# kzampog/cilantro

Hardware: NVIDIA H100
Metric: icp_correspondences_per_sec (higher is better)
Workload: dtype f32

## Files before the change

### cilantro_b200/capi.py

```python
import ctypes as C
import os
import weakref

import numpy as np

_HERE = os.path.dirname(os.path.abspath(__file__))
LIB_PATH = os.environ.get("CILANTRO_B200_LIB", os.path.join(_HERE, "libcilantro_b200.so"))

CB_OK = 0


class CbError(RuntimeError):
    pass


class IcpParams(C.Structure):
    _fields_ = [
        ("metric", C.c_int32),
        ("max_iter", C.c_int32),
        ("tol", C.c_float),
        ("max_d2", C.c_float),
        ("w_pt", C.c_float),
        ("w_pl", C.c_float),
        ("max_opt_iter", C.c_int32),
# ... 611 lines not shown
        n = lib().cb_icp_iteration_times(self.h, _p(times), C.c_int(times.shape[0]))
        return {
            "T": np.array(list(res.T), np.float32).reshape(3, 4),
            "iterations": int(res.iterations),
            "last_delta": float(res.last_delta),
            "converged": bool(res.converged),
            "num_corr": int(res.num_corr),
            "gpu_ms_total": float(res.gpu_ms_total),
            "gpu_ms_search": float(res.gpu_ms_search),
            "iter_ms": times[:max(n, 0)],
            "kernel_launches": int(res.kernel_launches),
        }

    def accumulate(self, T, **kw):
        prm = kw.pop("params", None) or icp_params(**kw)
        sums = np.zeros(28, np.float64)
        nv = _check(lib().cb_icp_accumulate(self.h, C.byref(prm), _p(_T(T)), _p(sums), C.c_int(28)))
        return sums[:nv]

    def correspondences(self):
        n = self.src.n + self.dst.n
        i1 = np.empty(n, np.uint64)
        i2 = np.empty(n, np.uint64)
        v = np.empty(n, np.float32)
        cnt = C.c_size_t()
        _check(lib().cb_icp_correspondences(self.h, _p(i1), _p(i2), _p(v), C.byref(cnt)))
        c = cnt.value
        return i1[:c].astype(np.int64), i2[:c].astype(np.int64), v[:c]

    def loop_cache(self):
        T = np.empty((3, 4), np.float32)
        near = np.empty(self.src.n, np.int64)
        cnt = C.c_uint64()
        _check(lib().cb_icp_loop_cache(self.h, _p(T), _p(near), C.byref(cnt)))
        return T, near, int(cnt.value)

    def residuals(self, T, **kw):
        prm = kw.pop("params", None) or icp_params(**kw)
        out = np.empty(self.src.n, np.float32)
        _check(lib().cb_icp_residuals(self.h, C.byref(prm), _p(_T(T)), _p(out)))
        return out


def solve_kabsch_moments(sums16):
    s = np.ascontiguousarray(sums16, np.float64)
    T = np.empty((3, 4), np.float32)
    ok = _check(lib().cb_solve_kabsch_moments(_p(s), _p(T)))
    return T, bool(ok)


def solve_gauss_newton(sums28, T_in=None):
    s = np.ascontiguousarray(sums28, np.float64)
    Ti = identity() if T_in is None else _T(T_in)
    To = np.empty((3, 4), np.float32)
    dn = C.c_float()
    _check(lib().cb_solve_gauss_newton(_p(s), _p(Ti), _p(To), C.byref(dn)))
    return To, dn.value


def solve_rotation(L):
    L = np.ascontiguousarray(L, np.float32).reshape(3, 3)
    R = np.empty((3, 3), np.float32)
    _check(lib().cb_solve_rotation(_p(L), _p(R)))
    return R


def compose(A, B):
    out = np.empty((3, 4), np.float32)
# ... 315 lines not shown
```

### cilantro_b200/csrc/capi_core.cu

```cuda
#include "cb_internal.hpp"
#include "icp_kernels.cuh"
#include "stats_kernels.cuh"
#include "host_solve.hpp"
#include "icp_object.hpp"
#include <atomic>
#include <cstdlib>
#include <cstring>
#include <cfloat>
#include <cmath>
#include <algorithm>
#include <vector>
#include <string>

namespace cb {

static thread_local std::string g_err;

void set_error(const char* fmt, ...) {
  char buf[1024];
  va_list ap;
  va_start(ap, fmt);
  vsnprintf(buf, sizeof(buf), fmt, ap);
  va_end(ap);
  g_err = buf;
// ... 875 lines not shown
    a.n_src = (uint32_t)ns;
    a.T = to_rigid(icp->T_search);
    a.Tin = to_rigid(nullptr);
    a.max_d2 = icp->max_d2_search;
    a.nn_pos = icp->d_nn_pos;
    a.nn_d2 = icp->d_nn_d2;
    CB_TRY(launch_icp_pass(ctx, a, kModeKnn, true, false, false));
    icp->nn_stored = true;
  }
  DeviceScope sc(ctx);
  int* d_first = nullptr;
  float* d_val = nullptr;
  CB_TRY(sc.alloc(&d_first, ns));
  CB_TRY(sc.alloc(&d_val, ns));
  CB_TRY(launch_translate_matches(ctx, icp->d_nn_pos, icp->d_nn_d2, icp->src->d_pts, icp->dst->d_pts, (uint32_t)ns, d_first,
                                  d_val));
  std::vector<int> first(ns);
  std::vector<float> val(ns);
  CB_CUDA(cudaMemcpyAsync(first.data(), d_first, ns * sizeof(int), cudaMemcpyDeviceToHost, ctx->stream));
  CB_CUDA(cudaMemcpyAsync(val.data(), d_val, ns * sizeof(float), cudaMemcpyDeviceToHost, ctx->stream));
  CB_CUDA(cudaStreamSynchronize(ctx->stream));
  size_t k = 0;
  for (size_t i = 0; i < ns; i++) {
    if (first[i] < 0) continue;
    if (index_first) index_first[k] = (uint64_t)first[i] + icp->dst->index_offset;
    if (index_second) index_second[k] = (uint64_t)i + icp->src->index_offset;
    if (value) value[k] = val[i];
    ++k;
  }
  *count = k;
  return CB_OK;
}

int cb_icp_loop_cache(cb_icp* icp, float* T_search12, int64_t* nearest, uint64_t* searched_last) {
  CB_CHECK(icp, CB_ERR_INVALID, "null argument");
  CB_CHECK(icp->loop_last && icp->h_state, CB_ERR_INVALID, "the last cb_icp_estimate did not run on the device loop");
  cb_context* ctx = icp->ctx;
  CB_CUDA(cudaSetDevice(ctx->device));
  const size_t ns = icp->src->n;
  if (T_search12) std::memcpy(T_search12, icp->T_search, sizeof(icp->T_search));
  if (searched_last) *searched_last = icp->searched_last;
  if (nearest && ns) {
    DeviceScope sc(ctx);
    int* d_first = nullptr;
    CB_TRY(sc.alloc(&d_first, ns));
    CB_TRY(launch_translate_matches(ctx, icp->d_nn_pos, nullptr, icp->src->d_pts, icp->dst->d_pts, (uint32_t)ns, d_first,
                                    nullptr));
    std::vector<int> first(ns);
    CB_CUDA(cudaMemcpyAsync(first.data(), d_first, ns * sizeof(int), cudaMemcpyDeviceToHost, ctx->stream));
    CB_CUDA(cudaStreamSynchronize(ctx->stream));
    for (size_t i = 0; i < ns; i++) nearest[i] = first[i] < 0 ? -1 : (int64_t)first[i] + (int64_t)icp->dst->index_offset;
  }
  return CB_OK;
}

int cb_icp_residuals(cb_icp* icp, const cb_icp_params* prm, const float* T12, float* out) {
  CB_CHECK(icp && prm && T12 && out, CB_ERR_INVALID, "null argument");
  cb_context* ctx = icp->ctx;
  CB_CUDA(cudaSetDevice(ctx->device));
  const size_t ns = icp->src->n;
  if (ns == 0) return CB_OK;
  CB_CHECK(prm->metric == CB_ICP_POINT_TO_POINT || icp->dst->d_nrm || icp->dst->n == 0, CB_ERR_INVALID,
           "dst has no normals");
  DeviceScope scope(ctx);
  float* d_out = nullptr;
  CB_TRY(scope.alloc(&d_out, ns));
  CB_TRY(launch_residuals(ctx, grid_view(icp->dst), icp->src->d_pts,
                          prm->metric == CB_ICP_COMBINED ? icp->src->d_nrm : nullptr, (uint32_t)ns, to_rigid(T12),
                          prm->metric, prm->w_pt, prm->w_pl, d_out));
  CB_CUDA(cudaMemcpyAsync(out, d_out, ns * sizeof(float), cudaMemcpyDeviceToHost, ctx->stream));
  CB_CUDA(cudaStreamSynchronize(ctx->stream));
  return CB_OK;
}

}
```

### cilantro_b200/csrc/icp_loop.cu

```cuda
#include "cache_rule.hpp"
#include "icp_accumulate.cuh"
#include "icp_kernels.cuh"
#include "icp_object.hpp"
#include "reduce.cuh"
#include "solve_core.hpp"
#include "solve_warp.cuh"
#include "warp_search_wide.cuh"
#include <algorithm>
#include <cmath>
#include <cstdlib>
#include <cstring>

namespace cb {

namespace {

constexpr int kBlock = kReduceBlock;

struct LoopArgs {
  GridView dst;
  const float4* src_pts;
  const float4* src_nrm;
  uint32_t n_src;
  float max_d2, w_pt, w_pl, tol;
  int wk_pt, wk_pl;
  float wc_pt, wc_pl;
  float dm[3];
  float src_mean[3];
  int has_pt, has_pl;
  int bail;
  int* cache_pos;
  float* cache_r;
  float slack_first, slack_min, slack_max;
  LoopState* st;
  ReduceScratch rs;
  int trace;
};

struct BlockCtx {
  Rigid T, Tp;
  float dm[3], sm[3];
  float w_pt, w_pl;
  int wk_pt, wk_pl;
  float wc_pt, wc_pl;
  int have_prev, done;
};

__device__ __forceinline__ Rigid rigid_from_t12_dev(const float* T12) {
  Rigid r;
#pragma unroll
  for (int i = 0; i < 3; i++) {
#pragma unroll
    for (int j = 0; j < 3; j++) r.r[i * 3 + j] = __ldcg(T12 + i * 4 + j);
    r.t[i] = __ldcg(T12 + i * 4 + 3);
  }
  return r;
}

template <int MODE>
__device__ __forceinline__ void loop_solve(const LoopArgs* ap, const BlockCtx* cxp, const double* s, int late,
                                        unsigned long long seq) {
  const LoopArgs& a = *ap;
  const BlockCtx& cx = *cxp;
  LoopState* st = a.st;
  if (late) {
    st->error = CB_ERR_NCCL;
// ... 20 lines not shown
    }
  }
  sc::reorthonormalize(Titer);
  sc::compose(Titer, T, Tn);
  const float delta = sc::update_norm(Titer);
  for (int i = 0; i < 12; i++) {
    st->T_prev[i] = T[i];
    st->T[i] = Tn[i];
    st->Titer[i] = Titer[i];
  }
  for (int i = 0; i < 28; i++) st->sums[i] = (i < (MODE == kModeP2PCentered ? kP2PValues : kCombinedValues)) ? s[i] : 0.0;
  st->last_delta = delta;
  st->iters = st->iters + 1;
  st->n_corr = s[0];
  st->have_prev = 1;
  st->xseq = seq;
  st->searched_last = st->searched_cur;
  st->searched_cur = 0ull;
  if (delta < a.tol) st->done = 1;
  if (a.trace) {
    st->trace[(st->iters - 1) & 63][3] = global_timer_ns();
    st->trace[st->iters & 63][5] = 0ull;
  }
  __threadfence();
}

struct ChunkPair {
  uint32_t i;
  int pos;
  float qx, qy, qz;
  float d2;
};

constexpr unsigned int kColdGroup = 1, kWarmGroup = 2;
template <bool kCold>
__device__ __forceinline__ ChunkPair search_chunk_body(const LoopArgs& a, const BlockCtx& cx, WideSearchSmem* wsm,
                                                       bool act, uint32_t i) {
  ChunkPair cp;
  cp.i = i;
  cp.pos = -1;
  cp.qx = cp.qy = cp.qz = 0.f;
  cp.d2 = 0.f;
  float slack = a.slack_first;
  int sd = -1;
  if (act) {
    const float4 s = __ldg(a.src_pts + cp.i);
    rule::transform_point(cx.T, s.x, s.y, s.z, cp.qx, cp.qy, cp.qz);
    if (!kCold) {
      float ox, oy, oz;
      rule::transform_point(cx.Tp, s.x, s.y, s.z, ox, oy, oz);
      const float ex = __fsub_rn(cp.qx, ox), ey = __fsub_rn(cp.qy, oy), ez = __fsub_rn(cp.qz, oz);
      const float dl = __fsqrt_ru(__fmaf_ru(ez, ez, __fmaf_ru(ey, ey, __fmul_ru(ex, ex))));
      slack = fminf(fmaxf(__fmul_rn(2.f, dl), a.slack_min), a.slack_max);
      sd = a.cache_pos[cp.i];
    }
  }
  const WideBest wb = warp_grid_nearest_wide<kCold ? kColdGroup : kWarmGroup>(a.dst, *wsm, act, cp.qx, cp.qy, cp.qz, a.max_d2, sd, slack);
  if (act) {
    cp.pos = (wb.idx >= 0 && wb.d2 < a.max_d2) ? wb.pos : -1;
    cp.d2 = wb.d2;
    a.cache_pos[cp.i] = cp.pos;
    a.cache_r[cp.i] = rule::cache_radius(wb.D2);
  }
  return cp;
}

__device__ __noinline__ void search_chunk_far(const LoopArgs* ap, const BlockCtx* cxp, WideSearchSmem* wsm, bool act,
                                              uint32_t i, ChunkPair* out) {
  *out = search_chunk_body<false>(*ap, *cxp, wsm, act, i);
}

__device__ __forceinline__ void pdl_wait() { asm volatile("griddepcontrol.wait;" ::: "memory"); }
__device__ __forceinline__ void pdl_launch_dependents() { asm volatile("griddepcontrol.launch_dependents;" ::: "memory"); }

__device__ __forceinline__ void load_block_ctx(const LoopArgs& a, BlockCtx& cx) {
  cx.done = __ldcg(&a.st->done);
  cx.have_prev = __ldcg(&a.st->have_prev);
  cx.T = rigid_from_t12_dev(a.st->T);
  cx.Tp = rigid_from_t12_dev(a.st->T_prev);
  float smx, smy, smz;
  rule::transform_point(cx.T, a.src_mean[0], a.src_mean[1], a.src_mean[2], smx, smy, smz);
  cx.sm[0] = smx; cx.sm[1] = smy; cx.sm[2] = smz;
  cx.dm[0] = a.dm[0]; cx.dm[1] = a.dm[1]; cx.dm[2] = a.dm[2];
  cx.w_pt = a.w_pt;
  cx.w_pl = a.w_pl;
  cx.wk_pt = a.wk_pt;
  cx.wk_pl = a.wk_pl;
  cx.wc_pt = a.wc_pt;
  cx.wc_pl = a.wc_pl;
}

__host__ __device__ constexpr int pipe_qpt(bool normals) { return normals ? 2 : 1; }
__host__ __device__ constexpr int pipe_min_blocks(bool normals) { return normals ? 2 : 4; }

__device__ __forceinline__ uint32_t smem_u32(const void* p) { return (uint32_t)__cvta_generic_to_shared(p); }
__device__ __forceinline__ void cp_async_16_cg(void* dst_smem, const void* src) {
  asm volatile("cp.async.cg.shared.global [%0], [%1], 16;" ::"r"(smem_u32(dst_smem)), "l"(src) : "memory");
}
__device__ __forceinline__ void cp_async_16_ca(void* dst_smem, const void* src) {
  asm volatile("cp.async.ca.shared.global [%0], [%1], 16;" ::"r"(smem_u32(dst_smem)), "l"(src) : "memory");
}
__device__ __forceinline__ void cp_async_4(void* dst_smem, const void* src) {
// ... 140 lines not shown
      const unsigned int mm = __ballot_sync(0xffffffffu, miss);
      const unsigned int at = queued + __popc(mm & ((1u << lane) - 1u));
      if (miss && at < 32u) wq[at] = i;
      queued += __popc(mm);
      if (queued >= 32u) {
        search_queued(32u);
        queued -= 32u;
        if (miss && at >= 32u) wq[at - 32u] = i;
      }
    }
    abuf = abuf1;
    bbuf ^= 1;
  }
  cp_async_wait<0>();
  if (queued > 0u) search_queued(queued);
  if (lane == 0 && searched > 0u) {
    atomicAdd(&a.st->searched_cur, (unsigned long long)searched);
    if (a.trace) atomicAdd(&a.st->trace[__ldcg(&a.st->iters) & 63][4], (unsigned long long)searched);
  }
  if (a.trace && lane == 0) atomicMax(&a.st->trace[__ldcg(&a.st->iters) & 63][5], global_timer_ns());
  warp_sum_to_slot<NV, true>(acc, rsm);
  double tot = 0;
  if (!grid_reduce_slots_tail<NV>(a.rs, rsm, tot)) return;
  if (lane < NV) a.rs.result[lane] = tot;
  if (a.trace && lane == 0) a.st->trace[__ldcg(&a.st->iters) & 63][1] = global_timer_ns();
}

constexpr int kSearchMinBlocks = 4;

template <int MODE>
__global__ void __launch_bounds__(kBlock, kSearchMinBlocks) icp_search_kernel(const __grid_constant__ LoopArgs a) {
  constexpr int NV = (MODE == kModeP2PCentered) ? kP2PValues : kCombinedValues;
  __shared__ BlockCtx cx;
  __shared__ WideSearchSmem wsm[kBlock / 32];
  __shared__ AsyncReduceSmem<NV> rsm;

  const unsigned int tid = threadIdx.x, lane = tid & 31u, warp = tid >> 5;
  const uint32_t base = blockIdx.x * kBlock;
  pdl_wait();
  pdl_launch_dependents();
  if (tid == 0) {
    rsm.arrived = 0u;
    load_block_ctx(a, cx);
  }
  __syncthreads();
  if (cx.done) return;
  const int trace_slot = a.trace ? (__ldcg(&a.st->iters) & 63) : 0;
  if (a.trace && blockIdx.x == 0 && tid == 0) {
    a.st->trace[trace_slot][0] = global_timer_ns();
    a.st->trace[trace_slot][4] = 0ull;
  }
  const unsigned int total = (base < a.n_src) ? min((uint32_t)kBlock, a.n_src - base) : 0u;
  if (tid == 0 && total > 0) {
    atomicAdd(&a.st->searched_cur, (unsigned long long)total);
    if (a.trace) atomicAdd(&a.st->trace[trace_slot][4], (unsigned long long)total);
  }
  double acc[NV];
#pragma unroll
  for (int v = 0; v < NV; v++) acc[v] = 0.0;
  if ((tid & ~31u) < total) {
    const ChunkPair cp = search_chunk_body<true>(a, cx, &wsm[warp], tid < total, base + tid);
    if (cp.pos >= 0) {
      const float4 dp = __ldg(a.dst.pts + cp.pos);
      accumulate_pair<MODE, true>(
          acc, cx, a.has_pt != 0, a.has_pl != 0, dp, cp.qx, cp.qy, cp.qz, a.src_nrm != nullptr,
          [&] { return __ldg(a.dst.nrm + cp.pos); }, [&] { return __ldg(a.src_nrm + cp.i); }, cp.d2);
    }
  }
  if (a.trace && lane == 0) atomicMax(&a.st->trace[trace_slot][5], global_timer_ns());
  double tot = 0;
  if (!grid_reduce_async_tail<NV>(acc, a.rs, rsm, tot)) return;
  if (lane < NV) a.rs.result[lane] = tot;
  if (a.trace && lane == 0) a.st->trace[trace_slot][1] = global_timer_ns();
}

template <int MODE>
__global__ void __launch_bounds__(32, 1) icp_finish_kernel(const __grid_constant__ LoopArgs a) {
  constexpr int NV = (MODE == kModeP2PCentered) ? kP2PValues : kCombinedValues;
  __shared__ BlockCtx cx;
  __shared__ double sbuf[kCombinedValues + 8];
  static_assert(NV + 2 <= kExchangeVals, "row of the fused exchange");
  const unsigned int lane = threadIdx.x;
  pdl_wait();
  pdl_launch_dependents();
  if (lane == 0) load_block_ctx(a, cx);
  __syncwarp();
  if (cx.done) return;
  const int trace_slot = a.trace ? (__ldcg(&a.st->iters) & 63) : 0;
  double tot = (lane < NV) ? __ldcg(a.rs.result + lane) : 0.0;
  if (lane == NV) tot = (double)__ldcg(&a.st->searched_cur);
  if (lane == NV + 1) tot = (double)a.n_src;
  bool late = false;
  const unsigned long long seq = __ldcg(&a.st->xseq) + 1ull;
  if (a.rs.ex.enabled && a.rs.ex.world > 1) {
    Exchange ex = a.rs.ex;
    ex.seq = seq;
    tot = exchange_rows<NV + 2>(tot, ex, (int)lane, &late);
  }
  if (lane == NV) a.st->searched_all = tot;
  if (lane == NV + 1) a.st->queries_all = tot;
  if (a.trace && lane == 0) a.st->trace[trace_slot][2] = global_timer_ns();
  if (lane < NV) sbuf[lane] = tot;
  __syncwarp();
  if constexpr (MODE == kModeCombined) {
    double x[6];
    solve6_warp(sbuf, (int)lane, x);
    if (lane == 0)
#pragma unroll
      for (int i = 0; i < 6; i++) sbuf[kCombinedValues + i] = x[i];
    __syncwarp();
  }
  if (lane == 0) loop_solve<MODE>(&a, &cx, sbuf, late ? 1 : 0, seq);
}

}

constexpr float kSlackFirst = 0.20f, kSlackMin = 0.02f, kSlackMax = 0.30f;
constexpr int kBatch = 16;
constexpr int kFirstBatch = 4;
constexpr int kBridgeBatch = 2;
constexpr double kGiveUpShare = 0.15;

template <class Kernel>
static cudaError_t launch_pdl(Kernel k, int blocks, int threads, size_t smem, cudaStream_t stream, const LoopArgs& a) {
  cudaLaunchConfig_t cfg;
  std::memset(&cfg, 0, sizeof(cfg));
  cfg.gridDim = dim3((unsigned)blocks);
  cfg.blockDim = dim3((unsigned)threads);
  cfg.dynamicSmemBytes = smem;
  cfg.stream = stream;
  cudaLaunchAttribute attr[1];
  attr[0].id = cudaLaunchAttributeProgrammaticStreamSerialization;
  attr[0].val.programmaticStreamSerializationAllowed = 1;
  cfg.attrs = attr;
  cfg.numAttrs = 1;
  return cudaLaunchKernelEx(&cfg, k, a);
}

template <int MODE>
static int enqueue_iteration(cb_context* ctx, const LoopArgs& a, int it, int blocks_cold, int blocks_cached) {
  if (it == 0)
    CB_CUDA(launch_pdl(icp_search_kernel<MODE>, blocks_cold, kBlock, 0, ctx->stream, a));
  else
    CB_CUDA(launch_pdl(icp_cached_pipe_kernel<MODE>, blocks_cached, kBlock, sizeof(PipeSmem<MODE == kModeCombined>),
                       ctx->stream, a));
  CB_CUDA(launch_pdl(icp_finish_kernel<MODE>, 1, 32, 0, ctx->stream, a));
  ctx->launches += 2;
  return CB_OK;
}

// ... 6 lines not shown
  if (!icp->d_state) CB_TRY(icp->mem.alloc(&icp->d_state, 1));
  if (!icp->h_state) CB_TRY(icp->mem.alloc_host(&icp->h_state, 1));
  while (timing != 0 && (int)icp->events.size() < 2 * max_iter) {
    cudaEvent_t e;
    CB_CUDA(cudaEventCreate(&e));
    icp->events.push_back(e);
  }
  const size_t ns = icp->src->n;
  LoopArgs a;
  std::memset(&a, 0, sizeof(a));
  a.dst = grid_view(icp->dst);
  a.src_pts = icp->src->d_pts;
  a.src_nrm = (prm->metric == CB_ICP_COMBINED) ? icp->src->d_nrm : nullptr;
  a.n_src = (uint32_t)ns;
  a.max_d2 = prm->max_d2;
  a.w_pt = prm->w_pt;
  a.w_pl = prm->w_pl;
  a.wk_pt = prm->pt_weight_kind == CB_WEIGHT_RBF;
  a.wk_pl = prm->pl_weight_kind == CB_WEIGHT_RBF;
  a.wc_pt = prm->pt_weight_coeff;
  a.wc_pl = prm->pl_weight_coeff;
  a.tol = prm->tol;
  for (int r = 0; r < 3; r++) {
    a.dm[r] = icp->dst_mean[r];
    a.src_mean[r] = icp->src_mean[r];
  }
  const bool dst_has_normals = icp->dst->d_nrm != nullptr;
  a.has_pt = prm->w_pt > 0.f;
  a.has_pl = (prm->w_pl > 0.f) && dst_has_normals;
  a.bail = (prm->w_pl > 0.f) && !dst_has_normals;
  a.cache_pos = icp->d_nn_pos;
  a.cache_r = icp->d_nn_d2;
  const float h = 1.0f / a.dst.inv_h;
  a.slack_first = kSlackFirst * h;
  a.slack_min = kSlackMin * h;
  a.slack_max = kSlackMax * h;
  a.st = icp->d_state;
  static const bool trace = getenv("CB_LOOP_TRACE") != nullptr;
  a.trace = trace ? 1 : 0;
  const int blocks_cold = std::max(1, (int)((ns + kBlock - 1) / kBlock));
  static bool attr_set_dev[64] = {};
  static int resident_dev[64][2] = {};
  bool& attr_set = attr_set_dev[ctx->device & 63];
  int* resident = resident_dev[ctx->device & 63];
  if (!attr_set) {
    CB_CUDA(cudaFuncSetAttribute(icp_cached_pipe_kernel<kModeP2PCentered>, cudaFuncAttributeMaxDynamicSharedMemorySize,
                                 (int)sizeof(PipeSmem<false>)));
    CB_CUDA(cudaFuncSetAttribute(icp_cached_pipe_kernel<kModeCombined>, cudaFuncAttributeMaxDynamicSharedMemorySize,
                                 (int)sizeof(PipeSmem<true>)));
    CB_CUDA(cudaFuncSetAttribute(icp_cached_pipe_kernel<kModeP2PCentered>, cudaFuncAttributePreferredSharedMemoryCarveout,
                                 (int)cudaSharedmemCarveoutMaxShared));
    CB_CUDA(cudaFuncSetAttribute(icp_cached_pipe_kernel<kModeCombined>, cudaFuncAttributePreferredSharedMemoryCarveout,
                                 (int)cudaSharedmemCarveoutMaxShared));
    CB_CUDA(cudaOccupancyMaxActiveBlocksPerMultiprocessor(&resident[0], icp_cached_pipe_kernel<kModeP2PCentered>, kBlock,
                                                          sizeof(PipeSmem<false>)));
    CB_CUDA(cudaOccupancyMaxActiveBlocksPerMultiprocessor(&resident[1], icp_cached_pipe_kernel<kModeCombined>, kBlock,
                                                          sizeof(PipeSmem<true>)));
    attr_set = true;
  }
  const bool p2p = prm->metric == CB_ICP_POINT_TO_POINT;
  const int per_sm = std::max(1, resident[p2p ? 0 : 1]);
  const size_t tile = (size_t)pipe_qpt(!p2p) * kBlock;
  const int blocks_cached = std::max(1, std::min(ctx->sm_count * per_sm, (int)((ns + tile - 1) / tile)));
  CB_TRY(get_reduce_scratch(ctx, blocks_cold, kMaxValues, &a.rs));
  Exchange ex;
  std::memset(&ex, 0, sizeof(ex));
  const bool fused = ctx->world > 1 && arm_exchange(ctx, &ex);
  if (fused) ctx->seq -= 1;
  if (ctx->world > 1 && !fused) {
    set_error("the device-resident ICP loop needs the fused exchange (cb_comm_ipc_attach) when world > 1");
    return CB_ERR_UNSUPPORTED;
  }
  a.rs.ex = ex;
  ctx->pass_armed = false;

  LoopState* hs = icp->h_state;
  std::memset(hs, 0, sizeof(*hs));
  std::memcpy(hs->T, prm->T_init, sizeof(hs->T));
  std::memcpy(hs->T_prev, prm->T_init, sizeof(hs->T));
  hs->last_delta = INFINITY;
  hs->xseq = ctx->seq;
  CB_CUDA(cudaMemcpyAsync(icp->d_state, hs, sizeof(*hs), cudaMemcpyHostToDevice, ctx->stream));

  int issued = 0;
  if (!icp->h_state2) CB_TRY(icp->mem.alloc_host(&icp->h_state2, 1));
  for (int e = 0; e < 2; ++e)
    if (!icp->batch_ev[e]) CB_CUDA(cudaEventCreateWithFlags(&icp->batch_ev[e], cudaEventDisableTiming));
  LoopState* hbuf[2] = {icp->h_state, icp->h_state2};
  int enq = 0, checked = 0;
  auto enqueue_batch = [&](int n) -> int {
    for (int k = 0; k < n; ++k) {
      if (prm->flush_l2) CB_TRY(cb_context_flush_l2(ctx));
      if (timing) CB_CUDA(cudaEventRecord(icp->events[2 * (issued + k)], ctx->stream));
// ... 78 lines not shown
```

### cilantro_b200/csrc/nn_search.cuh

```cuda
#pragma once
#include "cache_rule.hpp"
#include "cb_internal.hpp"

namespace cb {

struct Rigid {
  float r[9];
  float t[3];
};

inline Rigid rigid_from_t12(const float* T12) {
  Rigid r;
  for (int i = 0; i < 3; i++) {
    for (int j = 0; j < 3; j++) r.r[i * 3 + j] = T12 ? T12[i * 4 + j] : (i == j ? 1.f : 0.f);
    r.t[i] = T12 ? T12[i * 4 + 3] : 0.f;
  }
  return r;
}

__device__ __forceinline__ float sum3(float a0, float a1, float a2) { return __fadd_rn(a0, __fadd_rn(a1, a2)); }

__device__ __forceinline__ void rotate_rigid(const Rigid& T, float x, float y, float z, float& qx, float& qy,
                                             float& qz) {
  qx = sum3(__fmul_rn(T.r[0], x), __fmul_rn(T.r[1], y), __fmul_rn(T.r[2], z));
// ... 83 lines not shown
      }
    }
  } else {
    scan_batched(pts, b, e, qx, qy, qz, [&](float r, uint32_t j) {
      if (r < best.d2) {
        best.d2 = r;
        best.pos = (int)j;
      } else if (r == best.d2 && (int)j != skip_pos) {
        best.tie = true;
      }
    });
  }
}

__device__ __forceinline__ float slab_gap(float f, int c, int r) {
  float g = 0.f;
  if (r > c) g = (float)r - f;
  if (r < c) g = f - (float)(r + 1);
  g -= kCellMargin;
  return g > 0.f ? g : 0.f;
}

__device__ __forceinline__ bool open_face_gap(const GridView& g, const QueryCell& c, int kk, float& gap) {
  float cover = 3.0e38f;
  bool any = false;
  if (c.cx - kk > 0) { cover = fminf(cover, c.fx - (float)(c.cx - kk)); any = true; }
  if (c.cx + kk < g.nx - 1) { cover = fminf(cover, (float)(c.cx + kk + 1) - c.fx); any = true; }
  if (c.cy - kk > 0) { cover = fminf(cover, c.fy - (float)(c.cy - kk)); any = true; }
  if (c.cy + kk < g.ny - 1) { cover = fminf(cover, (float)(c.cy + kk + 1) - c.fy); any = true; }
  if (c.cz - kk > 0) { cover = fminf(cover, c.fz - (float)(c.cz - kk)); any = true; }
  if (c.cz + kk < g.nz - 1) { cover = fminf(cover, (float)(c.cz + kk + 1) - c.fz); any = true; }
  gap = cover - kCellMargin;
  return any;
}

}

#include "far_sweep.cuh"

namespace cb {

template <bool kExact>
__device__ __forceinline__ Best grid_nearest_impl(const GridView& g, float qx, float qy, float qz, float max_d2) {
  Best best = no_best(max_d2);
  if (g.n == 0) return best;
  if (!(fabsf(qx) + fabsf(qy) + fabsf(qz) < 3.0e38f)) return best;

  const QueryCell c = query_cell(g, qx, qy, qz);
  const int cx = c.cx, cy = c.cy, cz = c.cz;
  const float hs2 = g.hs2;
  const int k0 = first_shell(g, c);
  int k = k0;
  if (k0 == 0) {
    const int xm = max(cx - 1, 0), xp = min(cx + 1, g.nx - 1);
    const uint32_t cbase = ((uint32_t)cz * (uint32_t)g.ny + (uint32_t)cy) * (uint32_t)g.nx;
    const uint32_t s0 = __ldg(g.cell_start + cbase + xm), s1 = __ldg(g.cell_start + cbase + cx);
    const uint32_t s2 = __ldg(g.cell_start + cbase + cx + 1), s3 = __ldg(g.cell_start + cbase + xp + 1);
    constexpr int kDy[8] = {-1, 1, 0, 0, -1, 1, -1, 1};
    constexpr int kDz[8] = {0, 0, -1, 1, -1, -1, 1, 1};
    uint32_t rb[8], re[8];
#pragma unroll
    for (int t = 0; t < 8; ++t) {
      const int ry = cy + kDy[t], rz = cz + kDz[t];
      const bool valid = (ry >= 0) & (ry < g.ny) & (rz >= 0) & (rz < g.nz);
      const uint32_t base = valid ? ((uint32_t)rz * (uint32_t)g.ny + (uint32_t)ry) * (uint32_t)g.nx : cbase;
      const uint32_t b = __ldg(g.cell_start + base + xm), e = __ldg(g.cell_start + base + xp + 1);
// ... 104 lines not shown
```

### cilantro_b200/csrc/warp_search_wide.cuh

```cuda
#pragma once
#include "warp_search.cuh"

namespace cb {

struct WideSearchSmem : WarpQueue {
  unsigned int sec[32];
};
static_assert(sizeof(WideSearchSmem) <= 3456, "WideSearchSmem must not grow");

struct WideBest {
  float d2;
  int idx;
  int pos;
  float D2;
};

__device__ __forceinline__ void two_smallest(float r, int j, float& b1, int& p1, float& b2) {
  if (r < b1) {
    b2 = b1;
    b1 = r;
    p1 = j;
  } else {
    b2 = fminf(b2, r);
  }
}

__device__ __forceinline__ void scan_range_two(const float4* __restrict__ pts, uint32_t b, uint32_t e, float qx, float qy,
                                               float qz, float& b1, int& p1, float& b2, int skip) {
  scan_batched(pts, b, e, qx, qy, qz, [&](float r, uint32_t j) {
    if ((int)j != skip) two_smallest(r, (int)j, b1, p1, b2);
  });
}

__device__ __forceinline__ void merge_region(WideSearchSmem& sm, unsigned int owner, float l1, int lp, float l2,
                                             float max_d2) {
  constexpr float kInf = 3.402823466e+38f;
  float loser = l1;
  if (l1 < max_d2) {
    const unsigned long long key = pack_key(l1, (unsigned int)lp);
    const unsigned long long old = atomicMin(&sm.key[owner], key);
    const float od2 = __uint_as_float((unsigned int)(old >> 32));
    loser = ((unsigned int)(old & 0xffffffffull) == 0xffffffffu) ? kInf : fmaxf(od2, l1);
  }
  atomicMin(&sm.sec[owner], __float_as_uint(fminf(l2, loser)));
}

template <unsigned int kGroup>
__device__ __forceinline__ WideBest warp_grid_nearest_wide(const GridView& g, WideSearchSmem& sm, bool active, float qx,
                                                           float qy, float qz, float max_d2, int warm_pos, float slack) {
  const unsigned int lane = threadIdx.x & 31;
  const unsigned int lt_mask = (1u << lane) - 1u;
  constexpr float kInf = 3.402823466e+38f;
  WideBest out;
  out.d2 = max_d2;
  out.idx = -1;
  out.pos = -1;
  out.D2 = 0.f;

  const QueryCell c = query_cell(g, qx, qy, qz);
  const bool inside = active && g.n > 0 && c.cx >= 0 && c.cx < g.nx && c.cy >= 0 && c.cy < g.ny && c.cz >= 0 && c.cz < g.nz;
  bool slow = active && g.n > 0 && !inside;

  float b1 = kInf, b2 = kInf;
  int p1 = -1;
  if (inside && warm_pos >= 0) {
    const float4 p = __ldg(g.pts + warm_pos);
    b1 = rule::contract_d2(qx, qy, qz, p.x, p.y, p.z);
    p1 = warm_pos;
  }
  sm.q[lane] = make_float4(qx, qy, qz, 0.f);
  __syncwarp();

  unsigned int count = 0;
  float wide2 = 0.f;
  {
    const uint32_t cbase = inside ? ((uint32_t)c.cz * (uint32_t)g.ny + (uint32_t)c.cy) * (uint32_t)g.nx : 0u;
    uint32_t s1 = 0, s2 = 0;
// ... 18 lines not shown
    for (int t = 0; t < 10; ++t) {
      bool need;
      uint32_t first;
      uint32_t ncells;
      if (t == 0) {
        need = inside && c.cx > 0 && (gxl * gxl * g.hs2 <= wide2);
        first = cbase + (uint32_t)(c.cx - 1);
        ncells = 1;
      } else if (t == 1) {
        need = inside && c.cx < g.nx - 1 && (gxr * gxr * g.hs2 <= wide2);
        first = cbase + (uint32_t)(c.cx + 1);
        ncells = 1;
      } else {
        const int ry = c.cy + kDy[t - 2], rz = c.cz + kDz[t - 2];
        const bool valid = inside && ry >= 0 && ry < g.ny && rz >= 0 && rz < g.nz;
        need = valid && ((gy2[kDy[t - 2] + 1] + gz2[kDz[t - 2] + 1]) * g.hs2 <= wide2);
        first = ((uint32_t)rz * (uint32_t)g.ny + (uint32_t)ry) * (uint32_t)g.nx + (uint32_t)xm;
        ncells = (uint32_t)(xp - xm + 1);
      }
      const unsigned int m = __ballot_sync(0xffffffffu, need);
      if (need) sm.item[count + __popc(m & lt_mask)] = make_uint2(first, (ncells << 8) | lane);
      count += __popc(m);
    }
    if (b1 < max_d2) {
      sm.key[lane] = pack_key(b1, (unsigned int)p1);
      sm.sec[lane] = __float_as_uint(b2);
    } else {
      sm.key[lane] = pack_key(max_d2, 0xffffffffu);
      sm.sec[lane] = __float_as_uint(b1);
    }
  }
  __syncwarp();

  static_assert(kGroup >= 1 && kGroup <= 32 && (kGroup & (kGroup - 1)) == 0, "lanes per region: a power of two");
  if constexpr (kGroup == 1) {
    for (unsigned int k = lane; k < count; k += 32) {
      const QueueItem it = queue_item(g, sm, k);
      if (it.b >= it.e) continue;
      const unsigned long long cur = sm.key[it.lane];
      float l1 = kInf, l2 = kInf;
      int lp = -1;
      scan_range_two(g.pts, it.b, it.e, it.q.x, it.q.y, it.q.z, l1, lp, l2, (int)(unsigned int)(cur & 0xffffffffull));
      if (lp < 0) continue;
      merge_region(sm, it.lane, l1, lp, l2, max_d2);
    }
  } else {
    const unsigned int sub = lane & (kGroup - 1u);
    for (unsigned int k0 = 0; k0 < count; k0 += 32u / kGroup) {
      const unsigned int k = k0 + lane / kGroup;
      float l1 = kInf, l2 = kInf;
      int lp = -1;
      unsigned int owner = 0;
      if (k < count) {
        const QueueItem it = queue_item(g, sm, k);
        owner = it.lane;
        const int skip = (int)(unsigned int)(sm.key[it.lane] & 0xffffffffull);
        for (uint32_t j = it.b + sub; j < it.e; j += 2u * kGroup) {
          const float4 p0 = __ldg(g.pts + j);
          const bool has1 = j + kGroup < it.e;
          float4 p1 = p0;
          if (has1) p1 = __ldg(g.pts + j + kGroup);
          const float r0 = rule::contract_d2(it.q.x, it.q.y, it.q.z, p0.x, p0.y, p0.z);
          if ((int)j != skip) two_smallest(r0, (int)j, l1, lp, l2);
          if (has1) {
            const float r1 = rule::contract_d2(it.q.x, it.q.y, it.q.z, p1.x, p1.y, p1.z);
            if ((int)(j + kGroup) != skip) two_smallest(r1, (int)(j + kGroup), l1, lp, l2);
          }
        }
      }
#pragma unroll
      for (unsigned int m = 1; m < kGroup; m <<= 1) {
        const float o1 = __shfl_xor_sync(0xffffffffu, l1, m), o2 = __shfl_xor_sync(0xffffffffu, l2, m);
        const int op = __shfl_xor_sync(0xffffffffu, lp, m);
        l2 = fminf(fmaxf(l1, o1), fminf(l2, o2));
        if (o1 < l1 || (o1 == l1 && op > lp)) {
          l1 = o1;
          lp = op;
        }
      }
      if (sub == 0 && lp >= 0) merge_region(sm, owner, l1, lp, l2, max_d2);
    }
  }
  __syncwarp();

  if (inside) {
    const unsigned long long key = sm.key[lane];
    const unsigned int pos = (unsigned int)(key & 0xffffffffull);
    out.d2 = __uint_as_float((unsigned int)(key >> 32));
    out.pos = (pos == 0xffffffffu) ? -1 : (int)pos;
    const float sec = __uint_as_float(sm.sec[lane]);
    float cover;
    const bool any = open_face_gap(g, c, 1, cover);
    const float cover2 = (!any) ? kInf : (cover > 0.f ? cover * cover * g.hs2 : 0.f);
    const bool done = cover2 > out.d2;
    const bool tie = out.pos >= 0 && sec == out.d2;
    if (!done || tie) slow = true;
    out.D2 = fminf(fminf(sec, wide2), cover2);
  }
  if (slow) {
    const Best bst = grid_nearest(g, qx, qy, qz, max_d2);
    out.d2 = bst.d2;
    out.idx = bst.idx;
    out.pos = bst.pos;
    out.D2 = 0.f;
  } else if (out.pos >= 0) {
    out.idx = __float_as_int(__ldg(&g.pts[out.pos].w));
  }
  __syncwarp();
  return out;
}

}
```

### include/cilantro_b200.h

```cpp
#ifndef CILANTRO_B200_H_
#define CILANTRO_B200_H_

#include <stddef.h>
#include <stdint.h>

#ifdef __cplusplus
extern "C" {
#endif
#if defined(__GNUC__)
#pragma GCC visibility push(default)
#endif

typedef enum cb_status {
  CB_OK = 0,
  CB_ERR_INVALID = -1,
  CB_ERR_NO_DEVICE = -2,
  CB_ERR_CUDA = -3,
  CB_ERR_NCCL = -4,
  CB_ERR_UNSUPPORTED = -5
} cb_status;

typedef struct cb_context cb_context;
typedef struct cb_cloud cb_cloud;
typedef struct cb_icp cb_icp;
// ... 116 lines not shown
  float pl_weight_coeff;
} cb_icp_params;

typedef enum cb_weight_kind { CB_WEIGHT_UNITY = 0, CB_WEIGHT_RBF = 1 } cb_weight_kind;

typedef enum cb_search_dir {
  CB_SECOND_TO_FIRST = 0,
  CB_FIRST_TO_SECOND = 1,
  CB_BOTH = 2
} cb_search_dir;

typedef struct cb_icp_result {
  float T[12];
  int32_t iterations;
  float last_delta;
  int32_t converged;
  uint64_t num_corr;
  double gpu_ms_total;
  double gpu_ms_search;
  uint64_t kernel_launches;
} cb_icp_result;

void cb_icp_default_params(cb_icp_params* p);
int cb_icp_create(cb_context* ctx, const cb_cloud* dst, const cb_cloud* src, cb_icp** out);
void cb_icp_destroy(cb_icp* icp);
int cb_icp_estimate(cb_icp* icp, const cb_icp_params* prm, cb_icp_result* res);
int cb_icp_iteration_times(cb_icp* icp, double* ms, int cap);
int cb_icp_correspondences(cb_icp* icp, uint64_t* index_first, uint64_t* index_second, float* value,
                           size_t* count);
int cb_icp_residuals(cb_icp* icp, const cb_icp_params* prm, const float* T12, float* out);

int cb_icp_accumulate(cb_icp* icp, const cb_icp_params* prm, const float* T12, double* sums, int cap);

int cb_icp_loop_cache(cb_icp* icp, float* T_search12, int64_t* nearest, uint64_t* searched_last);

int cb_solve_kabsch_moments(const double* sums16, float* T12);
int cb_solve_gauss_newton(const double* sums28, const float* T_in12, float* T_out12, float* dtheta_norm);
int cb_solve_rotation(const float* L9, float* R9);
int cb_compose(const float* A12, const float* B12, float* out12);

typedef struct cb_kmeans_result {
  uint64_t iterations;
  double gpu_ms_total;
  uint64_t kernel_launches;
} cb_kmeans_result;
int cb_kmeans_cluster(cb_context* ctx, const cb_cloud* pts, float* centroids, size_t k, size_t max_iter,
                      float tol, uint64_t* labels, cb_kmeans_result* res);
int cb_kmeans_assign(cb_context* ctx, const cb_cloud* pts, const float* centroids, size_t k, uint64_t* labels,
                     double* sums, uint64_t* counts);
int cb_kmeans_seed_indices(size_t n, size_t k, uint32_t seed, uint64_t* out_idx);

int cb_ransac_score(cb_context* ctx, const cb_cloud* dst, const cb_cloud* src, const float* T_h, size_t H,
                    float thresh, uint32_t* counts);
int cb_ransac_residuals(cb_context* ctx, const cb_cloud* dst, const cb_cloud* src, const float* T12,
                        float thresh, float* residuals, uint64_t* inliers, size_t* num_inliers);
typedef struct cb_ransac_result {
  float T[12];
  uint64_t iterations;
  uint64_t num_inliers;
  uint64_t best_iteration;
  double gpu_ms_total;
  uint64_t kernel_launches;
} cb_ransac_result;
int cb_ransac_rigid(cb_context* ctx, const cb_cloud* dst, const cb_cloud* src, uint32_t seed,
                    size_t inlier_count_thresh, size_t max_iter, float thresh, int re_estimate,
                    cb_ransac_result* res, uint64_t* inliers, float* residuals);

// ... 132 lines not shown
```

Measured before the change: 16.81 billion.

## Replace cold warp-cooperative search with per-lane 3x3x3 block scan over persistent tiles

The cold (first-iteration) ICP search kernel no longer uses the warp-cooperative wide search with slack. Each lane now scans the 27 neighbouring grid cells itself as nine x-row ranges, falling back to the full grid search when the cover test fails. For point-to-point the kernel runs a grid capped at SM-resident blocks that loop over tiles, accumulating into shared reduction slots per tile. This removes warp shared-memory queueing and block-count overhead, at the risk of lane divergence and more slow-path fallbacks. A radius readback option is added to the loop cache API.

Result: no change. 16.95 billion (median of 6 runs) (+0.9%).

```diff
diff --git a/cilantro_b200/capi.py b/cilantro_b200/capi.py
--- a/cilantro_b200/capi.py
+++ b/cilantro_b200/capi.py
@@ -667,8 +667,13 @@
         T = np.empty((3, 4), np.float32)
         near = np.empty(self.src.n, np.int64)
         cnt = C.c_uint64()
-        _check(lib().cb_icp_loop_cache(self.h, _p(T), _p(near), C.byref(cnt)))
+        _check(lib().cb_icp_loop_cache(self.h, _p(T), _p(near), C.byref(cnt), None))
         return T, near, int(cnt.value)
+
+    def loop_radius(self):
+        r = np.empty(self.src.n, np.float32)
+        _check(lib().cb_icp_loop_cache(self.h, None, None, None, _p(r)))
+        return r
 
     def residuals(self, T, **kw):
         prm = kw.pop("params", None) or icp_params(**kw)
diff --git a/cilantro_b200/csrc/capi_core.cu b/cilantro_b200/csrc/capi_core.cu
--- a/cilantro_b200/csrc/capi_core.cu
+++ b/cilantro_b200/csrc/capi_core.cu
@@ -931,7 +931,7 @@
   return CB_OK;
 }
 
-int cb_icp_loop_cache(cb_icp* icp, float* T_search12, int64_t* nearest, uint64_t* searched_last) {
+int cb_icp_loop_cache(cb_icp* icp, float* T_search12, int64_t* nearest, uint64_t* searched_last, float* radius) {
   CB_CHECK(icp, CB_ERR_INVALID, "null argument");
   CB_CHECK(icp->loop_last && icp->h_state, CB_ERR_INVALID, "the last cb_icp_estimate did not run on the device loop");
   cb_context* ctx = icp->ctx;
@@ -939,16 +939,20 @@
   const size_t ns = icp->src->n;
   if (T_search12) std::memcpy(T_search12, icp->T_search, sizeof(icp->T_search));
   if (searched_last) *searched_last = icp->searched_last;
-  if (nearest && ns) {
+  if ((nearest || radius) && ns) {
     DeviceScope sc(ctx);
     int* d_first = nullptr;
+    float* d_r = nullptr;
     CB_TRY(sc.alloc(&d_first, ns));
-    CB_TRY(launch_translate_matches(ctx, icp->d_nn_pos, nullptr, icp->src->d_pts, icp->dst->d_pts, (uint32_t)ns, d_first,
-                                    nullptr));
+    if (radius) CB_TRY(sc.alloc(&d_r, ns));
+    CB_TRY(launch_translate_matches(ctx, icp->d_nn_pos, radius ? icp->d_nn_d2 : nullptr, icp->src->d_pts,
+                                    icp->dst->d_pts, (uint32_t)ns, d_first, d_r));
     std::vector<int> first(ns);
     CB_CUDA(cudaMemcpyAsync(first.data(), d_first, ns * sizeof(int), cudaMemcpyDeviceToHost, ctx->stream));
+    if (radius) CB_CUDA(cudaMemcpyAsync(radius, d_r, ns * sizeof(float), cudaMemcpyDeviceToHost, ctx->stream));
     CB_CUDA(cudaStreamSynchronize(ctx->stream));
-    for (size_t i = 0; i < ns; i++) nearest[i] = first[i] < 0 ? -1 : (int64_t)first[i] + (int64_t)icp->dst->index_offset;
+    if (nearest)
+      for (size_t i = 0; i < ns; i++) nearest[i] = first[i] < 0 ? -1 : (int64_t)first[i] + (int64_t)icp->dst->index_offset;
   }
   return CB_OK;
 }
diff --git a/cilantro_b200/csrc/icp_loop.cu b/cilantro_b200/csrc/icp_loop.cu
--- a/cilantro_b200/csrc/icp_loop.cu
+++ b/cilantro_b200/csrc/icp_loop.cu
@@ -31,7 +31,7 @@
   int bail;
   int* cache_pos;
   float* cache_r;
-  float slack_first, slack_min, slack_max;
+  float slack_min, slack_max;
   LoopState* st;
   ReduceScratch rs;
   int trace;
@@ -118,42 +118,42 @@
   float d2;
 };
 
-constexpr unsigned int kColdGroup = 1, kWarmGroup = 2;
-template <bool kCold>
-__device__ __forceinline__ ChunkPair search_chunk_body(const LoopArgs& a, const BlockCtx& cx, WideSearchSmem* wsm,
-                                                       bool act, uint32_t i) {
+__device__ __forceinline__ int cache_search_result(const LoopArgs& a, uint32_t i, const WideBest& wb) {
+  const int pos = (wb.idx >= 0 && wb.d2 < a.max_d2) ? wb.pos : -1;
+  a.cache_pos[i] = pos;
+  a.cache_r[i] = rule::cache_radius(wb.D2);
+  return pos;
+}
+
+constexpr unsigned int kWarmGroup = 2;
+
+__device__ __noinline__ void search_chunk_far(const LoopArgs* ap, const BlockCtx* cxp, WideSearchSmem* wsm, bool act,
+                                              uint32_t i, ChunkPair* out) {
+  const LoopArgs& a = *ap;
+  const BlockCtx& cx = *cxp;
   ChunkPair cp;
   cp.i = i;
   cp.pos = -1;
   cp.qx = cp.qy = cp.qz = 0.f;
   cp.d2 = 0.f;
-  float slack = a.slack_first;
+  float slack = 0.f;
   int sd = -1;
   if (act) {
     const float4 s = __ldg(a.src_pts + cp.i);
     rule::transform_point(cx.T, s.x, s.y, s.z, cp.qx, cp.qy, cp.qz);
-    if (!kCold) {
-      float ox, oy, oz;
-      rule::transform_point(cx.Tp, s.x, s.y, s.z, ox, oy, oz);
-      const float ex = __fsub_rn(cp.qx, ox), ey = __fsub_rn(cp.qy, oy), ez = __fsub_rn(cp.qz, oz);
-      const float dl = __fsqrt_ru(__fmaf_ru(ez, ez, __fmaf_ru(ey, ey, __fmul_ru(ex, ex))));
-      slack = fminf(fmaxf(__fmul_rn(2.f, dl), a.slack_min), a.slack_max);
-      sd = a.cache_pos[cp.i];
-    }
-  }
-  const WideBest wb = warp_grid_nearest_wide<kCold ? kColdGroup : kWarmGroup>(a.dst, *wsm, act, cp.qx, cp.qy, cp.qz, a.max_d2, sd, slack);
+    float ox, oy, oz;
+    rule::transform_point(cx.Tp, s.x, s.y, s.z, ox, oy, oz);
+    const float ex = __fsub_rn(cp.qx, ox), ey = __fsub_rn(cp.qy, oy), ez = __fsub_rn(cp.qz, oz);
+    const float dl = __fsqrt_ru(__fmaf_ru(ez, ez, __fmaf_ru(ey, ey, __fmul_ru(ex, ex))));
+    slack = fminf(fmaxf(__fmul_rn(2.f, dl), a.slack_min), a.slack_max);
+    sd = a.cache_pos[cp.i];
+  }
+  const WideBest wb = warp_grid_nearest_wide<kWarmGroup>(a.dst, *wsm, act, cp.qx, cp.qy, cp.qz, a.max_d2, sd, slack);
   if (act) {
-    cp.pos = (wb.idx >= 0 && wb.d2 < a.max_d2) ? wb.pos : -1;
+    cp.pos = cache_search_result(a, cp.i, wb);
     cp.d2 = wb.d2;
-    a.cache_pos[cp.i] = cp.pos;
-    a.cache_r[cp.i] = rule::cache_radius(wb.D2);
-  }
-  return cp;
-}
-
-__device__ __noinline__ void search_chunk_far(const LoopArgs* ap, const BlockCtx* cxp, WideSearchSmem* wsm, bool act,
-                                              uint32_t i, ChunkPair* out) {
-  *out = search_chunk_body<false>(*ap, *cxp, wsm, act, i);
+  }
+  *out = cp;
 }
 
 __device__ __forceinline__ void pdl_wait() { asm volatile("griddepcontrol.wait;" ::: "memory"); }
@@ -360,11 +360,9 @@
 __global__ void __launch_bounds__(kBlock, kSearchMinBlocks) icp_search_kernel(const __grid_constant__ LoopArgs a) {
   constexpr int NV = (MODE == kModeP2PCentered) ? kP2PValues : kCombinedValues;
   __shared__ BlockCtx cx;
-  __shared__ WideSearchSmem wsm[kBlock / 32];
   __shared__ AsyncReduceSmem<NV> rsm;
 
-  const unsigned int tid = threadIdx.x, lane = tid & 31u, warp = tid >> 5;
-  const uint32_t base = blockIdx.x * kBlock;
+  const unsigned int tid = threadIdx.x, lane = tid & 31u;
   pdl_wait();
   pdl_launch_dependents();
   if (tid == 0) {
@@ -378,26 +376,40 @@
     a.st->trace[trace_slot][0] = global_timer_ns();
     a.st->trace[trace_slot][4] = 0ull;
   }
-  const unsigned int total = (base < a.n_src) ? min((uint32_t)kBlock, a.n_src - base) : 0u;
-  if (tid == 0 && total > 0) {
-    atomicAdd(&a.st->searched_cur, (unsigned long long)total);
-    if (a.trace) atomicAdd(&a.st->trace[trace_slot][4], (unsigned long long)total);
-  }
-  double acc[NV];
-#pragma unroll
-  for (int v = 0; v < NV; v++) acc[v] = 0.0;
-  if ((tid & ~31u) < total) {
-    const ChunkPair cp = search_chunk_body<true>(a, cx, &wsm[warp], tid < total, base + tid);
-    if (cp.pos >= 0) {
-      const float4 dp = __ldg(a.dst.pts + cp.pos);
-      accumulate_pair<MODE, true>(
-          acc, cx, a.has_pt != 0, a.has_pl != 0, dp, cp.qx, cp.qy, cp.qz, a.src_nrm != nullptr,
-          [&] { return __ldg(a.dst.nrm + cp.pos); }, [&] { return __ldg(a.src_nrm + cp.i); }, cp.d2);
-    }
+  const uint32_t ntiles = (a.n_src + kBlock - 1) / kBlock;
+  const uint32_t t0 = (uint32_t)(((uint64_t)ntiles * blockIdx.x) / gridDim.x);
+  const uint32_t t1 = (uint32_t)(((uint64_t)ntiles * (blockIdx.x + 1)) / gridDim.x);
+  const uint32_t first = t0 * kBlock, last = min(t1 * kBlock, a.n_src);
+  if (tid == 0 && last > first) {
+    atomicAdd(&a.st->searched_cur, (unsigned long long)(last - first));
+    if (a.trace) atomicAdd(&a.st->trace[trace_slot][4], (unsigned long long)(last - first));
+  }
+  const unsigned int warp = tid >> 5;
+  if (lane < NV) rsm.slot[warp][lane] = 0.0;
+  __syncwarp();
+#pragma unroll 1
+  for (uint32_t i = first + tid; i - tid < last; i += kBlock) {
+    double acc[NV];
+#pragma unroll
+    for (int v = 0; v < NV; v++) acc[v] = 0.0;
+    if (i < last) {
+      const float4 s = __ldg(a.src_pts + i);
+      float qx, qy, qz;
+      rule::transform_point(cx.T, s.x, s.y, s.z, qx, qy, qz);
+      const WideBest wb = lane_block_nearest(a.dst, qx, qy, qz, a.max_d2);
+      const int pos = cache_search_result(a, i, wb);
+      if (pos >= 0) {
+        const float4 dp = __ldg(a.dst.pts + pos);
+        accumulate_pair<MODE, true>(
+            acc, cx, a.has_pt != 0, a.has_pl != 0, dp, qx, qy, qz, a.src_nrm != nullptr,
+            [&] { return __ldg(a.dst.nrm + pos); }, [&] { return __ldg(a.src_nrm + i); }, wb.d2);
+      }
+    }
+    warp_sum_to_slot<NV, true>(acc, rsm);
   }
   if (a.trace && lane == 0) atomicMax(&a.st->trace[trace_slot][5], global_timer_ns());
   double tot = 0;
-  if (!grid_reduce_async_tail<NV>(acc, a.rs, rsm, tot)) return;
+  if (!grid_reduce_slots_tail<NV>(a.rs, rsm, tot)) return;
   if (lane < NV) a.rs.result[lane] = tot;
   if (a.trace && lane == 0) a.st->trace[trace_slot][1] = global_timer_ns();
 }
@@ -443,7 +455,7 @@
 
 }
 
-constexpr float kSlackFirst = 0.20f, kSlackMin = 0.02f, kSlackMax = 0.30f;
+constexpr float kSlackMin = 0.02f, kSlackMax = 0.30f;
 constexpr int kBatch = 16;
 constexpr int kFirstBatch = 4;
 constexpr int kBridgeBatch = 2;
@@ -516,13 +528,11 @@
   a.cache_pos = icp->d_nn_pos;
   a.cache_r = icp->d_nn_d2;
   const float h = 1.0f / a.dst.inv_h;
-  a.slack_first = kSlackFirst * h;
   a.slack_min = kSlackMin * h;
   a.slack_max = kSlackMax * h;
   a.st = icp->d_state;
   static const bool trace = getenv("CB_LOOP_TRACE") != nullptr;
   a.trace = trace ? 1 : 0;
-  const int blocks_cold = std::max(1, (int)((ns + kBlock - 1) / kBlock));
   static bool attr_set_dev[64] = {};
   static int resident_dev[64][2] = {};
   bool& attr_set = attr_set_dev[ctx->device & 63];
@@ -543,6 +553,8 @@
     attr_set = true;
   }
   const bool p2p = prm->metric == CB_ICP_POINT_TO_POINT;
+  const int ntiles_cold = std::max(1, (int)((ns + kBlock - 1) / kBlock));
+  const int blocks_cold = p2p ? std::min(ntiles_cold, ctx->sm_count * kSearchMinBlocks) : ntiles_cold;
   const int per_sm = std::max(1, resident[p2p ? 0 : 1]);
   const size_t tile = (size_t)pipe_qpt(!p2p) * kBlock;
   const int blocks_cached = std::max(1, std::min(ctx->sm_count * per_sm, (int)((ns + tile - 1) / tile)));
diff --git a/cilantro_b200/csrc/nn_search.cuh b/cilantro_b200/csrc/nn_search.cuh
--- a/cilantro_b200/csrc/nn_search.cuh
+++ b/cilantro_b200/csrc/nn_search.cuh
@@ -139,6 +139,12 @@
   if (c.cz + kk < g.nz - 1) { cover = fminf(cover, (float)(c.cz + kk + 1) - c.fz); any = true; }
   gap = cover - kCellMargin;
   return any;
+}
+
+__device__ __forceinline__ float open_face_d2(const GridView& g, const QueryCell& c, int kk) {
+  float cover;
+  if (!open_face_gap(g, c, kk, cover)) return 3.402823466e+38f;
+  return cover > 0.f ? cover * cover * g.hs2 : 0.f;
 }
 
 }
diff --git a/cilantro_b200/csrc/warp_search_wide.cuh b/cilantro_b200/csrc/warp_search_wide.cuh
--- a/cilantro_b200/csrc/warp_search_wide.cuh
+++ b/cilantro_b200/csrc/warp_search_wide.cuh
@@ -43,6 +43,62 @@
     loser = ((unsigned int)(old & 0xffffffffull) == 0xffffffffu) ? kInf : fmaxf(od2, l1);
   }
   atomicMin(&sm.sec[owner], __float_as_uint(fminf(l2, loser)));
+}
+
+__device__ __forceinline__ bool block_scan_final(const GridView& g, const QueryCell& c, float d2, int pos, float sec,
+                                                 float& D2) {
+  const float cover2 = open_face_d2(g, c, 1);
+  D2 = fminf(sec, cover2);
+  const bool tie = pos >= 0 && sec == d2;
+  return cover2 > d2 && !tie;
+}
+
+__device__ __forceinline__ void finish_search(const GridView& g, bool slow, float qx, float qy, float qz, float max_d2,
+                                              WideBest& out) {
+  if (slow) {
+    const Best bst = grid_nearest(g, qx, qy, qz, max_d2);
+    out.d2 = bst.d2;
+    out.idx = bst.idx;
+    out.pos = bst.pos;
+    out.D2 = 0.f;
+  } else if (out.pos >= 0) {
+    out.idx = __float_as_int(__ldg(&g.pts[out.pos].w));
+  }
+}
+
+__device__ __forceinline__ WideBest lane_block_nearest(const GridView& g, float qx, float qy, float qz, float max_d2) {
+  constexpr float kInf = 3.402823466e+38f;
+  WideBest out;
+  out.d2 = max_d2;
+  out.idx = -1;
+  out.pos = -1;
+  out.D2 = 0.f;
+  if (g.n == 0) return out;
+  const QueryCell c = query_cell(g, qx, qy, qz);
+  bool slow = true;
+  if (c.cx >= 0 && c.cx < g.nx && c.cy >= 0 && c.cy < g.ny && c.cz >= 0 && c.cz < g.nz) {
+    const int xm = max(c.cx - 1, 0), xp = min(c.cx + 1, g.nx - 1);
+    uint32_t rb[9], re[9];
+#pragma unroll
+    for (int t = 0; t < 9; ++t) {
+      const int ry = c.cy + t % 3 - 1, rz = c.cz + t / 3 - 1;
+      const bool valid = ry >= 0 && ry < g.ny && rz >= 0 && rz < g.nz;
+      const uint32_t base = ((uint32_t)rz * (uint32_t)g.ny + (uint32_t)ry) * (uint32_t)g.nx;
+      rb[t] = valid ? __ldg(g.cell_start + base + xm) : 0u;
+      re[t] = valid ? __ldg(g.cell_start + base + xp + 1) : 0u;
+    }
+    float b1 = kInf, b2 = kInf;
+    int p1 = -1;
+#pragma unroll
+    for (int t = 0; t < 9; ++t) scan_range_two(g.pts, rb[t], re[t], qx, qy, qz, b1, p1, b2, -1);
+    if (b1 < max_d2) {
+      out.d2 = b1;
+      out.pos = p1;
+    }
+    slow = !block_scan_final(g, c, out.d2, out.pos, out.pos >= 0 ? b2 : b1, out.D2);
+  }
+  finish_search(g, slow, qx, qy, qz, max_d2, out);
+  return out;
 }
 
 template <unsigned int kGroup>
@@ -127,19 +183,8 @@
   }
   __syncwarp();
 
-  static_assert(kGroup >= 1 && kGroup <= 32 && (kGroup & (kGroup - 1)) == 0, "lanes per region: a power of two");
-  if constexpr (kGroup == 1) {
-    for (unsigned int k = lane; k < count; k += 32) {
-      const QueueItem it = queue_item(g, sm, k);
-      if (it.b >= it.e) continue;
-      const unsigned long long cur = sm.key[it.lane];
-      float l1 = kInf, l2 = kInf;
-      int lp = -1;
-      scan_range_two(g.pts, it.b, it.e, it.q.x, it.q.y, it.q.z, l1, lp, l2, (int)(unsigned int)(cur & 0xffffffffull));
-      if (lp < 0) continue;
-      merge_region(sm, it.lane, l1, lp, l2, max_d2);
-    }
-  } else {
+  static_assert(kGroup >= 2 && kGroup <= 32 && (kGroup & (kGroup - 1)) == 0, "lanes per region: a power of two");
+  {
     const unsigned int sub = lane & (kGroup - 1u);
     for (unsigned int k0 = 0; k0 < count; k0 += 32u / kGroup) {
       const unsigned int k = k0 + lane / kGroup;
@@ -184,23 +229,11 @@
     out.d2 = __uint_as_float((unsigned int)(key >> 32));
     out.pos = (pos == 0xffffffffu) ? -1 : (int)pos;
     const float sec = __uint_as_float(sm.sec[lane]);
-    float cover;
-    const bool any = open_face_gap(g, c, 1, cover);
-    const float cover2 = (!any) ? kInf : (cover > 0.f ? cover * cover * g.hs2 : 0.f);
-    const bool done = cover2 > out.d2;
-    const bool tie = out.pos >= 0 && sec == out.d2;
-    if (!done || tie) slow = true;
-    out.D2 = fminf(fminf(sec, wide2), cover2);
-  }
-  if (slow) {
-    const Best bst = grid_nearest(g, qx, qy, qz, max_d2);
-    out.d2 = bst.d2;
-    out.idx = bst.idx;
-    out.pos = bst.pos;
-    out.D2 = 0.f;
-  } else if (out.pos >= 0) {
-    out.idx = __float_as_int(__ldg(&g.pts[out.pos].w));
-  }
+    float D2;
+    if (!block_scan_final(g, c, out.d2, out.pos, sec, D2)) slow = true;
+    out.D2 = fminf(D2, wide2);
+  }
+  finish_search(g, slow, qx, qy, qz, max_d2, out);
   __syncwarp();
   return out;
 }
diff --git a/include/cilantro_b200.h b/include/cilantro_b200.h
--- a/include/cilantro_b200.h
+++ b/include/cilantro_b200.h
@@ -172,7 +172,7 @@
 
 int cb_icp_accumulate(cb_icp* icp, const cb_icp_params* prm, const float* T12, double* sums, int cap);
 
-int cb_icp_loop_cache(cb_icp* icp, float* T_search12, int64_t* nearest, uint64_t* searched_last);
+int cb_icp_loop_cache(cb_icp* icp, float* T_search12, int64_t* nearest, uint64_t* searched_last, float* radius);
 
 int cb_solve_kabsch_moments(const double* sums16, float* T12);
 int cb_solve_gauss_newton(const double* sums28, const float* T_in12, float* T_out12, float* dtheta_norm);
```
